# lucabaldesi/srsRAN

Measured on AMD Instinct MI355X. Metric: PDSCH decoded Mbps + code-blocks/sec, 20 MHz TM4 QAM256, 1/2/4/8 GPU, higher is better.
Workload: dtype fp32+int16; 1 GPU; srslte_ue_dl chain from time-domain I/Q: 2048 subframes/GPU/batch, 20 MHz (100 PRB), TM4 2x2 spatial multiplexing, 2 codewords QAM256 TBS 97896 (C=16, K=6144), MMSE+CSI, max 10 half-its with CRC early stop, 40 dB crossed 2x2 channel, every subframe distinct (GPU eNodeB generator, keyed by global subframe index); 3 PHY worker threads (own ue_dl / stream / softbuffers each) decode alternate batches,; subframes_per_gpu_batch=2048, code_blocks_per_gpu_batch=65536, workers_per_gpu=3, parallelism=dp1

## Files before the change

srsran_amd/csrc/tdec_internal.h:

```cpp
#pragma once
#include <hip/hip_runtime.h>
#include <stdint.h>

#include "dlsch_internal.h"

#define TDEC_INF 10000
#define TDEC_WARMUP 40
#define TDEC_SEG 8

namespace mi355 {

struct TdecWinArgs {
  const int16_t*  in;
  size_t          in_stride;
  const uint32_t* in_idx;
  const uint8_t*  done;
  const uint32_t* remaining;
  uint32_t*       A1;
  uint32_t*       E;
  uint32_t*       D;
  uint32_t*       ckpt;
  const uint32_t* dstE;
  const uint32_t* dstA;
  int             ncb, L, Lp, nseg, n, write_d;
  uint8_t*        dec;
  size_t          dec_stride;
  const uint32_t* gS;
  const uint32_t* gP;
  DlschCheckArgs  chk;
  int             chk_on;
  int             spec;
  int             rowmask;
};

struct TdecDecideArgs {
  const uint32_t* D;
  uint8_t*        out;
  size_t          out_stride;
  int             ncb, L, Lp;
  const uint8_t*  done;
  const uint32_t* remaining;
};

struct TdecGenArgs {
  const uint32_t* S;
  const uint32_t* P0;
  const uint32_t* P1;
  uint32_t*       A1;
  uint32_t*       E;
  uint32_t*       D;
  uint32_t*       ckpt;
  const uint16_t* pi;
  int             npair, K, Kp, nseg, n, write_d;
};

struct TdecGenPrepArgs {
  const int16_t*  in;
  size_t          stride;
  const uint32_t* in_idx;
  uint32_t *     S, *P0, *P1, *E;
  int            ncb, npair, K, Kp;
};

struct TdecGenDecideArgs {
  const uint32_t* D;
  uint8_t*        out;
  size_t          out_stride;
  int             ncb, K, Kp;
};

#define TDEC_GEN_CB_L 12
#define TDEC_GEN_CB_KP(K) (((K) + 3 + 7) / 8 * 8)
struct TdecGenCbArgs {
  const int16_t*  in;
  size_t          in_stride;
  const uint32_t* in_idx;
  uint16_t*       ws;
  const uint16_t* pi;
  uint8_t*        out;
  size_t          out_stride;
  uint32_t*       reruns;
  int             ncb, K, Kp, h0, h1, warm, persist;
};
int        tdec_gen_cb_threads(int K);
size_t     tdec_gen_cb_lds(int K, int threads);
hipError_t tdec_gen_cb_launch(const TdecGenCbArgs& a, hipStream_t s);

struct TdecLatArgs {
  const int16_t*  in;
  size_t          in_stride;
  const uint32_t* in_idx;
  const uint32_t* dstE;
  const uint32_t* dstA;
  uint8_t*        done;
  DlschCheckArgs  chk;
  uint64_t*       prof;
  int             ncb, K, rowmask;
  int             bwave;
  int             owaves;
};
size_t     tdec_lat_lds(int K, int nsb);
hipError_t tdec_lat_launch(int nsb, const TdecLatArgs& a, hipStream_t s);

struct TdecRun {
  const int16_t*  in;
  size_t          in_stride;
  const uint32_t* in_idx;
  const uint8_t*  done;
  const uint32_t* remaining;
  uint32_t        n, K, h0, h1;
  uint8_t*        out;
  size_t          out_stride;
  hipStream_t     stream;
  const DlschCheckArgs* chk = nullptr;
  bool*                 chk_fused = nullptr;
  bool  spec       = false;
  bool* spec_taken = nullptr;
  bool  redo       = false;
  bool  rowmask    = false;
};

hipError_t tdec_win_launch_halfit(int nsb, const TdecWinArgs& a, hipStream_t s);
bool       tdec_win_spec_ok(int nsb, int L);
int        tdec_set_diag(int mode);
hipError_t tdec_win_launch_decide(int nsb, const TdecDecideArgs& a, hipStream_t s);
hipError_t tdec_gen_launch_prep(const TdecGenPrepArgs& a, hipStream_t s);
hipError_t tdec_gen_launch_halfit(const TdecGenArgs& a, hipStream_t s);
hipError_t tdec_gen_launch_decide(const TdecGenDecideArgs& a, hipStream_t s);

}

struct mi355_tdec_batch;
int mi355_tdec_run_internal(mi355_tdec_batch* q, const mi355::TdecRun& r);
int mi355_tdec_win_tables(mi355_tdec_batch* q, uint32_t K, const uint32_t** dstE, const uint32_t** dstA);
```

srsran_amd/csrc/tdec_kernels.hip:

```cpp
#include <hip/hip_runtime.h>

#include <atomic>
#include <stdint.h>
#include <stdlib.h>

#include "crc_device.h"
#include "tdec_internal.h"
#include "tdec_trellis.h"

namespace mi355 {

__device__ __forceinline__ uint32_t hi_lo(uint32_t a, uint32_t b) { return __builtin_amdgcn_alignbit(b, a, 16); }
__device__ __forceinline__ uint32_t from_prev(uint32_t v)
{
  return (uint32_t)__builtin_amdgcn_update_dpp(0, (int)v, 0x111, 0xf, 0xf, true);
}
__device__ __forceinline__ uint32_t from_next(uint32_t v)
{
  return (uint32_t)__builtin_amdgcn_update_dpp(0, (int)v, 0x101, 0xf, 0xf, true);
}

__device__ __forceinline__ void bm_set(uint32_t* bm, uint32_t m, bool v)
{
  const uint32_t by = m >> 3;
  if (v) atomicOr(&bm[by >> 2], 1u << (((by & 3) << 3) + 7 - (m & 7)));
}

template <int NL>
__device__ __forceinline__ void tdec_fused_check(const TdecWinArgs& a, int cb, int l, int K, const uint32_t* bm,
                                                 const uint32_t (*t4)[4][256])
{
  const DlschCheckArgs& c      = a.chk;
  const CbDesc&         d      = c.desc[cb];
  const uint32_t        nbytes = (uint32_t)K / 8, chunk = nbytes / NL;
  const int             pi     = d.C > 1 ? 1 : 0;
  const uint8_t*        bytes  = (const uint8_t*)bm;
  uint32_t              crc    = crc24_words(bytes + l * chunk, chunk, t4[pi]);
  crc = gf2_mulmod24(crc, c.scale[128 + 8 * pi + l], pi ? c.crc24b->poly : c.crc24a->poly);
#pragma unroll
  for (int o = NL / 2; o >= 1; o >>= 1) crc ^= (uint32_t)__shfl_xor((int)crc, o, 64);
  const bool ok  = crc == 0;
  const bool fin = ok || c.h + 1 == c.max_its;
  if (fin) {
    uint8_t*       dst  = c.data + d.data_off + (size_t)d.cb * d.rlen / 8;
    const uint32_t nb   = d.nb;
    const uint32_t head = min(nb, (4u - (uint32_t)((uintptr_t)dst & 3u)) & 3u);
    const uint32_t nw   = (nb - head) / 4, tail0 = head + 4 * nw;
    for (uint32_t i = l; i < head; i += NL) dst[i] = bytes[i];
    for (uint32_t i = tail0 + l; i < nb; i += NL) dst[i] = bytes[i];
    uint32_t* dw = (uint32_t*)(dst + head);
    const uint32_t sh = head;
    for (uint32_t w = l; w < nw; w += NL) {
      const uint32_t lo = bm[w + sh / 4], hi = bm[w + sh / 4 + 1];
      dw[w]             = sh ? __builtin_amdgcn_alignbyte(hi, lo, sh) : lo;
    }
    if (l == 0) {
      c.its[cb] = c.h + 1;
      if (ok) {
        c.done[cb]       = 1;
        c.sb_crc[d.slot] = 1;
      } else {
        c.done[cb] = 2;
      }
    }
  }
  const uint64_t un = __builtin_amdgcn_ballot_w64(l == 0 && !fin);
  if (un && (threadIdx.x & 63) == (uint32_t)__builtin_ctzll(un)) flag_set(c.next);
}


#define WG_AT(arr, j) (arr)[((size_t)grp * Lp + (j)) * 64 + q]

#define TDEC_BM_WORDS (8 * 193)
__shared__ uint32_t tdec_tx_lds[4][2][TDEC_SEG * 64];
__shared__ uint32_t tdec_ym_lds[4][8 * SB_ROWMASK_WORDS];
__shared__ uint32_t tdec_bm_lds[4 * TDEC_BM_WORDS];
__shared__ int16_t  tdec_stg_lds[4][TDEC_SEG * 128];
__shared__ uint32_t tdec_stg_row[4][TDEC_SEG];

#ifndef TDEC_WAVES_PER_EU
#define TDEC_WAVES_PER_EU 2
#endif
template <int NSB, int SEG, int MODE, int DIAG, bool FULL, int OUTK, bool GI = false, bool TX = false>
__device__ __forceinline__ void tdec_win_body(const TdecWinArgs& a, const int gl,
                                              const uint32_t (*crc_t4)[4][256] = nullptr)
{
  constexpr int NL = NSB / 2;
  constexpr int G  = 64 / NL;
  static_assert(!TX || (NSB == 16 && FULL && SEG == 8), "TX loads need 8-lane rows and whole 8-step segments");
  static_assert((DIAG >= 0 && DIAG <= 4) || DIAG == 20, "DIAG values the body knows");
  const int     grp = __builtin_amdgcn_readfirstlane(gl >> 6), q = gl & 63;
  const int     cbg = q / NL, l = q % NL;
  if constexpr (!TX) {
    if (grp * G + cbg >= a.ncb) return;
    if (a.done && a.done[grp * G + cbg]) return;
  }
  if (a.remaining && *a.remaining == 0) return;

  const int  L = a.L, Lp = a.Lp, nseg = a.nseg;
  constexpr bool CL     = DIAG == 20;
  constexpr bool dec2   = MODE == 2;
  constexpr bool has_ap = MODE == 1;

  const int       cb   = grp * G + cbg;
  const int       K    = L * NSB;
  const size_t    bidx = a.in_idx ? a.in_idx[cb] : (size_t)cb;
  const uint32_t* in32 = (const uint32_t*)(a.in + bidx * a.in_stride);
  const size_t    wg0  = (size_t)grp * Lp * 64 + q;
  const uint32_t* X    = dec2 ? a.E + wg0 : (GI ? a.gS + wg0 : in32 + l);
  const int       xs   = (dec2 || GI) ? 64 : NL;
  const uint32_t* Y    = GI ? a.gP + wg0 : in32 + (dec2 ? (K + 32) : (K + 32) / 2) + l;
  const int       ys   = GI ? 64 : NL;
  const uint32_t* AP   = a.A1 + wg0;
  uint32_t*       ck   = a.ckpt + (size_t)grp * nseg * 8 * 64 + q;

  const uint4*    txin  = nullptr;
  if constexpr (TX) {
    const int txc = grp * G + ((q >> 1) & 7);
    txin = (const uint4*)(a.in + (a.in_idx ? (size_t)a.in_idx[txc] : (size_t)txc) * a.in_stride) + (2 * (q >> 4) + (q & 1));
  }
  const int       txoX  = 0;
  const int       txoY  = (dec2 ? (L * NSB + 32) : (L * NSB + 32) / 2) / 4;
  uint32_t*       txb   = nullptr;
  if constexpr (TX) {
    txb = &tdec_tx_lds[threadIdx.x >> 6][0][0];
  }
  constexpr bool RMK = NSB == 16 && !GI;
  uint32_t*      ymask = nullptr;
  if constexpr (RMK) {
    ymask = tdec_ym_lds[threadIdx.x >> 6];
#pragma unroll
    for (int w = l; w < SB_ROWMASK_WORDS; w += NL) {
      uint32_t v = 0xffffffffu;
      if (a.rowmask) v = ((const uint32_t*)(a.in + bidx * a.in_stride + SB_ROWMASK))[(dec2 ? SB_ROWMASK_WORDS : 0) + w];
      ymask[cbg * SB_ROWMASK_WORDS + w] = v;
    }
    __builtin_amdgcn_fence(__ATOMIC_RELEASE, "wavefront");
    __builtin_amdgcn_wave_barrier();
    __builtin_amdgcn_fence(__ATOMIC_ACQUIRE, "wavefront");
  }
  auto yrow = [&](int c, int j) -> bool {
    if constexpr (RMK) {
      return (ymask[c * SB_ROWMASK_WORDS + (j >> 5)] >> (j & 31)) & 1u;
    } else {
      return true;
    }
  };
  auto tx_load = [&](int so, int j0, uint32_t* r, bool par = false) {
    uint4 v0 = make_uint4(0u, 0u, 0u, 0u), v1 = v0;
    const int tc = (q >> 1) & 7, jr = j0 + (q >> 4);
    if (!par || yrow(tc, jr)) v0 = txin[so + j0 * 2];
    if (!par || yrow(tc, jr + 4)) v1 = txin[so + (j0 + 4) * 2];
    r[0] = v0.x; r[1] = v0.y; r[2] = v0.z; r[3] = v0.w;
    r[4] = v1.x; r[5] = v1.y; r[6] = v1.z; r[7] = v1.w;
  };
  auto tx_unpack = [&](int b, const uint32_t* r, uint32_t* o) {
    uint32_t* w = txb + b * SEG * 64;
    ((uint4*)w)[q]      = make_uint4(r[0], r[1], r[2], r[3]);
    ((uint4*)w)[64 + q] = make_uint4(r[4], r[5], r[6], r[7]);
    __builtin_amdgcn_fence(__ATOMIC_RELEASE, "wavefront");
    __builtin_amdgcn_wave_barrier();
    __builtin_amdgcn_fence(__ATOMIC_ACQUIRE, "wavefront");
#pragma unroll
    for (int i = 0; i < SEG; i++) o[i] = w[64 * i + q];
  };

  v2s st[8], nw[8], aw[8];

  set_minf(aw);
#pragma unroll 1
  for (int b = 0; b < TDEC_WARMUP / 8; b++) {
    uint32_t xo[8], yo[8], ao[8] = {};
#pragma unroll
    for (int i = 0; i < 8; i++) {
      const int j = (L - TDEC_WARMUP) + 8 * b + i;
      xo[i]       = X[j * xs];
      yo[i]       = yrow(cbg, j) ? Y[j * ys] : 0u;
      if constexpr (has_ap) ao[i] = AP[j * 64];
    }
#pragma unroll
    for (int i = 0; i < 8; i++) {
      const int k = 8 * b + i;
      v2s       x = U(hi_lo(from_prev(xo[i]), xo[i]));
      if constexpr (has_ap) x = sadd(x, U(hi_lo(from_prev(ao[i]), ao[i])));
      if constexpr (CL) {
        aw[k & 7] = aw[k & 7] ^ x ^ U(yo[i]);
        continue;
      }
      v2s c0[8], c1[8];
      alpha_cands<true>(aw, x, U(hi_lo(from_prev(yo[i]), yo[i])), c0, c1);
#pragma unroll
      for (int s = 0; s < 8; s++) aw[s] = vmax(c0[s], c1[s]);
      if ((k & 1) == 0 && k != 0) normalize<true>(aw);
    }
  }

  if constexpr (DIAG != 2) {
  set_minf(st);
#pragma unroll 1
  for (int b = TDEC_WARMUP / 8 - 1; b >= 0; b--) {
    uint32_t xo[8], yo[8], ao[8] = {};
#pragma unroll
    for (int i = 0; i < 8; i++) {
      const int j = 8 * b + i;
      xo[i]       = X[j * xs];
      yo[i]       = yrow(cbg, j) ? Y[j * ys] : 0u;
      if constexpr (has_ap) ao[i] = AP[j * 64];
    }
#pragma unroll
    for (int i = 7; i >= 0; i--) {
      const int k = 8 * b + i;
      v2s       x = U(hi_lo(xo[i], from_next(xo[i])));
      if constexpr (has_ap) x = sadd(x, U(hi_lo(ao[i], from_next(ao[i]))));
      if constexpr (CL) {
        st[k & 7] = st[k & 7] ^ x ^ U(yo[i]);
        continue;
      }
      beta_step<true>(st, x, U(hi_lo(yo[i], from_next(yo[i]))), nw);
#pragma unroll
      for (int s = 0; s < 8; s++) st[s] = nw[s];
      if ((k & 1) == 0 && k != 0) normalize<true>(st);
    }
  }
  if (l == NL - 1) {
    const int16_t* T = a.in + bidx * a.in_stride + 3 * (K + 32) + (dec2 ? 6 : 0);
    v2s            tr[8], tn[8];
    tr[0] = splat(0);
#pragma unroll
    for (int i = 1; i < 8; i++) tr[i] = splat(-TDEC_INF);
#pragma unroll
    for (int t = 2; t >= 0; t--) {
      beta_step<false>(tr, splat(T[2 * t]), splat(T[2 * t + 1]), tn);
#pragma unroll
      for (int i = 0; i < 8; i++) tr[i] = tn[i];
    }
#pragma unroll
    for (int i = 0; i < 8; i++) st[i] = (v2s){st[i].x, tr[i].y};
  }
#pragma unroll
  for (int s = 0; s < 8; s++) ck[((size_t)(nseg - 1) * 8 + s) * 64] = W(st[s]);

  {
    uint32_t cx[SEG], cy[SEG], ca[SEG] = {};
    auto     load = [&](int t, uint32_t* x, uint32_t* y, uint32_t* ap) {
      if constexpr (TX) {
        if constexpr (!dec2) tx_load(txoX, t * SEG, x);
        tx_load(txoY, t * SEG, y, true);
      }
#pragma unroll
      for (int i = 0; i < SEG; i++) {
        const int j = FULL ? t * SEG + i : min(t * SEG + i, L - 1);
        if constexpr (!TX || dec2) x[i] = X[j * xs];
        if constexpr (!TX) y[i] = yrow(cbg, j) ? Y[j * ys] : 0u;
        if constexpr (has_ap) ap[i] = AP[j * 64];
      }
    };
    uint32_t bx[SEG], by[SEG], ba[SEG] = {}, dx[SEG], dy[SEG], da[SEG] = {};
    load(nseg - 1, cx, cy, ca);
    if (nseg > 1) load(nseg - 2, bx, by, ba);
    auto seg = [&](int t, const uint32_t* rx, const uint32_t* ry, const uint32_t* sa, uint32_t* lx, uint32_t* ly,
                   uint32_t* la) {
      uint32_t sx[SEG], sy[SEG];
      if constexpr (TX) {
        if constexpr (!dec2) tx_unpack(0, rx, sx);
        tx_unpack(1, ry, sy);
      }
#pragma unroll
      for (int i = 0; i < SEG; i++) {
        if constexpr (!TX || dec2) sx[i] = rx[i];
        if constexpr (!TX) sy[i] = ry[i];
      }
      if (t > 1) load(t - 2, lx, ly, la);
#pragma unroll
      for (int i = SEG - 1; i >= 0; i--) {
        const int k = t * SEG + i;
        if (FULL || k < L) {
          v2s x = U(sx[i]);
          if constexpr (has_ap) x = sadd(x, U(sa[i]));
          if constexpr (DIAG == 4) {
            st[0] = st[0] ^ x ^ U(sy[i]);
            continue;
          }
          if constexpr (CL) {
            st[i] = st[i] ^ x ^ U(sy[i]);
          } else {
            beta_step<true>(st, x, U(sy[i]), nw);
#pragma unroll
            for (int s = 0; s < 8; s++) st[s] = nw[s];
          }
          if (i == 0 && t > 0 && DIAG != 3) {
#pragma unroll
            for (int s = 0; s < 8; s++) ck[((size_t)(t - 1) * 8 + s) * 64] = W(st[s]);
          }
          if (!CL && (i & 1) == 0 && k != 0) normalize<true>(st);
        }
      }
    };
#pragma unroll 1
    for (int t = nseg - 1; t >= 0; t -= 3) {
      seg(t, cx, cy, ca, dx, dy, da);
      if (t >= 1) seg(t - 1, bx, by, ba, cx, cy, ca);
      if (t >= 2) seg(t - 2, dx, dy, da, bx, by, ba);
    }
  }
  }
  if constexpr (DIAG == 1 || DIAG == 3 || DIAG == 4) {
    if (st[0].x == 12345 && st[1].y == 777) a.D[q] = W(st[0]);
    return;
  }
#pragma unroll
  for (int s = 0; s < 8; s++) st[s] = aw[s];
  if (l == 0) {
    st[0].x = 0;
#pragma unroll
    for (int i = 1; i < 8; i++) st[i].x = -TDEC_INF;
  }

  int16_t*        E16  = (int16_t*)a.E + (size_t)grp * Lp * 128;
  int16_t*        A16  = (int16_t*)a.A1 + (size_t)grp * Lp * 128;
  int16_t*        D16  = (int16_t*)a.D + (size_t)grp * Lp * 128;
  const uint32_t* tab  = (dec2 ? a.dstA : a.dstE) + l;
  const int       lane0 = cbg * NL;
  constexpr bool  dec_o   = OUTK == 1 || OUTK == 3;
  constexpr bool  wr_bits = !dec2 && dec_o && FULL;
  constexpr bool  wr_bm   = dec_o && (dec2 || !FULL);
  constexpr bool  wr_d    = OUTK == 2;
  constexpr bool  wr_a1   = !(dec2 && OUTK == 3);
  constexpr bool  wr_e    = !(!dec2 && OUTK == 3);
  constexpr int BMW = NSB == 16 ? 193 : 25;
  uint32_t*     bm  = nullptr;
  if constexpr (dec2 || wr_bits || wr_bm) {
    static_assert(G * BMW <= TDEC_BM_WORDS, "decision bitmaps of a wave");
    bm = tdec_bm_lds + (threadIdx.x >> 6) * TDEC_BM_WORDS + cbg * BMW;
    if constexpr (wr_bm) {
      for (int w = l; w < K / 32; w += NL) bm[w] = 0;
      __builtin_amdgcn_fence(__ATOMIC_RELEASE, "wavefront");
      __builtin_amdgcn_wave_barrier();
    }
  }

  constexpr bool STG = FULL && !GI && (dec2 ? wr_a1 : wr_e);
  int16_t*       O16 = dec2 ? A16 : E16;
  int16_t*       stg = nullptr;
  uint32_t*      stg_row = nullptr;
  if constexpr (STG) {
    stg     = tdec_stg_lds[threadIdx.x >> 6];
    stg_row = tdec_stg_row[threadIdx.x >> 6];
  }
  auto put = [&](int i, uint32_t tb, v2s v) {
    if constexpr (STG) {
      stg[i * 128 + (tb & 127u) + 2 * lane0]         = v.x;
      stg[i * 128 + ((tb >> 16) & 127u) + 2 * lane0] = v.y;
      stg_row[i]                                     = (tb & 0xffffu) >> 7;
    } else {
      O16[(tb & 0xffffu) + lane0 * 2] = v.x;
      O16[(tb >> 16) + lane0 * 2]     = v.y;
    }
  };
  auto flush = [&]() {
    if constexpr (STG) {
      static_assert(SEG == 8 && NL % 4 == 0, "rows of 8 steps, whole 16-byte pieces per code block");
      constexpr int PPR = NL / 4;
      __builtin_amdgcn_fence(__ATOMIC_RELEASE, "wavefront");
      __builtin_amdgcn_wave_barrier();
      __builtin_amdgcn_fence(__ATOMIC_ACQUIRE, "wavefront");
#pragma unroll
      for (int k = 0; k < 2; k++) {
        const int      idx = k * NL + l, r = idx / PPR, pc = idx % PPR;
        const uint32_t jr  = stg_row[r];
        const uint4    v   = *(const uint4*)(stg + r * 128 + 2 * lane0 + pc * 8);
        *(uint4*)(O16 + (size_t)jr * 128 + 2 * lane0 + pc * 8) = v;
      }
      __builtin_amdgcn_fence(__ATOMIC_RELEASE, "wavefront");
      __builtin_amdgcn_wave_barrier();
    }
  };
  uint32_t cx[SEG], cy[SEG], ca[SEG] = {}, cd[SEG], cc[8];
  auto     load = [&](int t, uint32_t* x, uint32_t* y, uint32_t* ap, uint32_t* d, uint32_t* c) {
    if constexpr (TX) {
      if constexpr (!dec2) tx_load(txoX, t * SEG, x);
      tx_load(txoY, t * SEG, y, true);
    }
#pragma unroll
    for (int i = 0; i < SEG; i++) {
      const int j = FULL ? t * SEG + i : min(t * SEG + i, L - 1);
      if constexpr (!TX || dec2) x[i] = X[j * xs];
      if constexpr (!TX) y[i] = yrow(cbg, j) ? Y[j * ys] : 0u;
      if constexpr (has_ap) ap[i] = AP[j * 64];
      d[i] = tab[(size_t)j * NL];
    }
#pragma unroll
    for (int s = 0; s < 8; s++) c[s] = ck[((size_t)t * 8 + s) * 64];
  };
  load(0, cx, cy, ca, cd, cc);

  uint32_t nx[SEG], ny[SEG], na[SEG] = {}, nd[SEG], nc[8];
  auto fseg = [&](int t, const uint32_t* rx, const uint32_t* ry, const uint32_t* ca, const uint32_t* cd,
                  const uint32_t* cc, uint32_t* nx, uint32_t* ny, uint32_t* na, uint32_t* nd, uint32_t* nc) {
    uint32_t cx[SEG], cy[SEG];
    if constexpr (TX) {
      if constexpr (!dec2) tx_unpack(0, rx, cx);
      tx_unpack(1, ry, cy);
    }
#pragma unroll
    for (int i = 0; i < SEG; i++) {
      if constexpr (!TX || dec2) cx[i] = rx[i];
      if constexpr (!TX) cy[i] = ry[i];
    }
    const int s0 = t * SEG;
    const int e  = FULL ? s0 + SEG : ((s0 + SEG < L) ? s0 + SEG : L);
    uint32_t  bits = 0;
    if (t + 1 < nseg) load(t + 1, nx, ny, na, nd, nc);

    v2s xin[SEG];
#pragma unroll
    for (int i = 0; i < SEG; i++) {
      if constexpr (has_ap) {
        xin[i] = sadd(U(cx[i]), U(ca[i]));
      } else {
        xin[i] = U(cx[i]);
      }
    }

    static_assert(SEG == 8, "the rebuild keeps the 8 rows of a segment in registers");
    v2s ck8[8];
#pragma unroll
    for (int s = 0; s < 8; s++) ck8[s] = U(cc[s]);
    if constexpr (CL) {
#pragma unroll
      for (int i = 0; i < SEG; i++) {
        const int j = s0 + i;
        if (FULL ? i < SEG : j < e) {
          const v2s      out = xin[i] ^ U(cy[i]) ^ ck8[i] ^ st[i];
          const uint32_t tb  = cd[i];
          if constexpr (!dec2) {
            if constexpr (wr_e) put(i, tb, out);
            bits |= ((uint32_t)(out.x > 0) << (15 - i)) | ((uint32_t)(out.y > 0) << (7 - i));
            if constexpr (wr_bm) {
              bm_set(bm, 2 * l * L + j, out.x > 0);
              bm_set(bm, (2 * l + 1) * L + j, out.y > 0);
            }
          } else {
            if constexpr (wr_a1) put(i, tb, out);
            if constexpr (wr_bm) {
              const uint32_t jd = (tb & 0xffffu) >> 7, wlo = tb & 15u, whi = (tb >> 16) & 15u;
              bm_set(bm, wlo * L + jd, out.x > 0);
              bm_set(bm, whi * L + jd, out.y > 0);
            }
          }
        }
      }
    } else {
      v2s        cur[8], R[8][8];
      const bool ck_norm = (e & 1) == 0 && e != L;
#pragma unroll
      for (int s = 0; s < 8; s++) cur[s] = ck8[s];
      if (ck_norm) normalize<true>(cur);
#pragma unroll
      for (int i = SEG; i >= 1; i--) {
        const int j = s0 + i;
        if (FULL ? i == SEG : j == e) {
#pragma unroll
          for (int s = 0; s < 8; s++) R[i - 1][s] = ck8[s];
        } else if (FULL ? i < SEG : j < e) {
          v2s row[8];
          beta_step<true>(cur, xin[i], U(cy[i]), row);
#pragma unroll
          for (int s = 0; s < 8; s++) cur[s] = row[s];
#pragma unroll
          for (int s = 0; s < 8; s++) R[i - 1][s] = row[s];
          if ((j & 1) == 0) normalize<true>(cur);
        }
      }
#pragma unroll
      for (int i = 0; i < SEG; i++) {
        const int j = s0 + i;
        if (FULL ? i < SEG : j < e) {
          v2s c0[8], c1[8];
          alpha_cands<true>(st, xin[i], U(cy[i]), c0, c1);
          v2s t0[8], t1[8];
#pragma unroll
          for (int s = 0; s < 8; s++) {
            t0[s] = sadd(R[i][s], c0[s]);
            t1[s] = sadd(R[i][s], c1[s]);
          }
          const v2s m0 = vmax(vmax(vmax(t0[0], t0[1]), vmax(t0[2], t0[3])), vmax(vmax(t0[4], t0[5]), vmax(t0[6], t0[7])));
          const v2s m1 = vmax(vmax(vmax(t1[0], t1[1]), vmax(t1[2], t1[3])), vmax(vmax(t1[4], t1[5]), vmax(t1[6], t1[7])));
          const v2s out = ssub(m1, m0);
#pragma unroll
          for (int s = 0; s < 8; s++) st[s] = vmax(c0[s], c1[s]);
          if ((i & 1) == 0 && j != 0) normalize<true>(st);

          const uint32_t tb  = cd[i];
          const uint32_t olo = (tb & 0xffffu) + lane0 * 2, ohi = (tb >> 16) + lane0 * 2;
          if constexpr (!dec2) {
            if constexpr (wr_e) put(i, tb, has_ap ? out - U(ca[i]) : out);
            if constexpr (wr_d) WG_AT(a.D, j) = W(out);
            bits |= ((uint32_t)(out.x > 0) << (15 - i)) | ((uint32_t)(out.y > 0) << (7 - i));
            if constexpr (wr_bm) {
              bm_set(bm, 2 * l * L + j, out.x > 0);
              bm_set(bm, (2 * l + 1) * L + j, out.y > 0);
            }
          } else {
            if constexpr (wr_a1) put(i, tb, out - xin[i]);
            if constexpr (wr_bm) {
              const uint32_t jd = (tb & 0xffffu) >> 7, wlo = tb & 15u, whi = (tb >> 16) & 15u;
              bm_set(bm, wlo * L + jd, out.x > 0);
              bm_set(bm, whi * L + jd, out.y > 0);
            }
            if constexpr (wr_d) {
              D16[olo] = out.x;
              D16[ohi] = out.y;
            }
          }
        }
      }
    }
    flush();
    if constexpr (wr_bits) {
      uint8_t* bb = (uint8_t*)bm + (size_t)(2 * l) * (L / 8) + t;
      bb[0]       = (uint8_t)(bits >> 8);
      bb[L / 8]   = (uint8_t)bits;
    }
  };
#pragma unroll 1
  for (int t = 0; t < nseg; t += 2) {
    fseg(t, cx, cy, ca, cd, cc, nx, ny, na, nd, nc);
    if (t + 1 < nseg) fseg(t + 1, nx, ny, na, nd, nc, cx, cy, ca, cd, cc);
  }
  if constexpr (wr_bm || wr_bits) {
    __builtin_amdgcn_fence(__ATOMIC_RELEASE, "wavefront");
    __builtin_amdgcn_wave_barrier();
    __builtin_amdgcn_fence(__ATOMIC_ACQUIRE, "wavefront");
    if (crc_t4) {
      tdec_fused_check<NL>(a, cb, l, K, bm, crc_t4);
    } else {
      uint2* o = (uint2*)(a.dec + (size_t)cb * a.dec_stride);
      for (int w = l; w < K / 64; w += NL) o[w] = make_uint2(bm[2 * w], bm[2 * w + 1]);
    }
  }
}

template <int NSB, int SEG, int MODE, int DIAG = 0, bool FULL = false, int OUTK = 0, bool TX = false>
__global__ __launch_bounds__(256) __attribute__((amdgpu_waves_per_eu(TDEC_WAVES_PER_EU))) void tdec_win_halfit(TdecWinArgs a)
{
  const int gl = blockIdx.x * blockDim.x + threadIdx.x;
  const uint32_t (*t4)[4][256] = nullptr;
  if constexpr (OUTK == 1 || OUTK == 3) {
    __shared__ uint32_t crc_t4[2][4][256];
    if (a.chk_on) {
      if (a.remaining && *a.remaining == 0) return;
      const uint32_t ti = threadIdx.x;
      crc_t4[0][0][ti] = a.chk.crc24a->t[ti];
      crc_t4[1][0][ti] = a.chk.crc24b->t[ti];
      __syncthreads();
#pragma unroll
      for (int k = 1; k < 4; k++) {
        crc_t4[0][k][ti] = crc24_step_table(crc_t4[0][k - 1][ti], crc_t4[0][0]);
        crc_t4[1][k][ti] = crc24_step_table(crc_t4[1][k - 1][ti], crc_t4[1][0]);
        __syncthreads();
      }
      t4 = crc_t4;
    }
  }
  if constexpr (TX) {
    const int  cb  = (gl >> 6) * (128 / NSB) + (gl & 63) / (NSB / 2);
    const bool act = cb < a.ncb && !(a.done && a.done[cb]);
    if (__builtin_amdgcn_ballot_w64(act) == ~0ull) {
      tdec_win_body<NSB, SEG, MODE, DIAG, FULL, OUTK, false, true>(a, gl, t4);
      return;
    }
  }
  tdec_win_body<NSB, SEG, MODE, DIAG, FULL, OUTK>(a, gl, t4);
}


template <int NSB>
__global__ __launch_bounds__(256) void tdec_win_decide_rows(TdecDecideArgs a)
{
  constexpr int NL = NSB / 2;
  constexpr int G  = 64 / NL;
  const size_t  g  = (size_t)blockIdx.x * blockDim.x + threadIdx.x;
  const int     q  = (int)(g & 63);
  const size_t  r  = g >> 6;
  const int     nb = a.L / 8;
  const int     grp = (int)(r / nb), jb = (int)(r % nb);
  const int     cbg = q / NL, l = q % NL;
  const size_t  cb  = (size_t)grp * G + cbg;
  if (cb >= (size_t)a.ncb || (a.remaining && *a.remaining == 0) || (a.done && a.done[cb])) return;
  const uint32_t* D  = a.D + ((size_t)grp * a.Lp + 8 * jb) * 64 + q;
  uint32_t        lo = 0, hi = 0;
#pragma unroll
  for (int i = 0; i < 8; i++) {
    const v2s v = U(D[(size_t)i * 64]);
    lo |= (uint32_t)(v.x > 0) << (7 - i);
    hi |= (uint32_t)(v.y > 0) << (7 - i);
  }
  uint8_t* o = a.out + cb * a.out_stride;
  o[(2 * l) * nb + jb]     = (uint8_t)lo;
  o[(2 * l + 1) * nb + jb] = (uint8_t)hi;
}

template <int NSB>
__global__ __launch_bounds__(256) void tdec_win_decide(TdecDecideArgs a)
{
  constexpr int NL   = NSB / 2;
  constexpr int G    = 64 / NL;
  const size_t  g    = (size_t)blockIdx.x * blockDim.x + threadIdx.x;
  const int     K    = a.L * NSB;
  const int     nbyt = K / 8;
  const size_t  cb   = g / nbyt;
  if (cb >= (size_t)a.ncb || (a.remaining && *a.remaining == 0) || (a.done && a.done[cb])) return;
  const int      b   = (int)(g % nbyt);
  const int      grp = (int)(cb / G), cbg = (int)(cb % G);
  const int16_t* D16 = (const int16_t*)a.D + (size_t)grp * a.Lp * 128 + cbg * NL * 2;
  uint32_t       out = 0;
#pragma unroll
  for (int i = 0; i < 8; i++) {
    const int nat = 8 * b + i, w = nat / a.L, j = nat % a.L;
    out |= (uint32_t)(D16[(size_t)j * 128 + w] > 0) << (7 - i);
  }
  a.out[cb * a.out_stride + b] = (uint8_t)out;
}


static std::atomic<int> g_diag{-1};

static int diag_mode()
{
  int v = g_diag.load(std::memory_order_relaxed);
  if (v < 0) {
    const char* e = getenv("MI355_TDEC_DIAG");
    v             = e ? atoi(e) : 0;
    g_diag.store(v, std::memory_order_relaxed);
  }
  return v;
}

int tdec_set_diag(int mode)
{
  const int old = diag_mode();
  g_diag.store(mode < 0 ? 0 : mode, std::memory_order_relaxed);
  return old;
}

static size_t diag_lds()
{
  static const long m = getenv("MI355_TDEC_LDS") ? atol(getenv("MI355_TDEC_LDS")) : 0;
  return (size_t)m;
}

template <int NSB, int DIAG, bool FULL, int OUTK, bool TX = false>
static void launch_mode_t(int mode, int blocks, const TdecWinArgs& a, hipStream_t s)
{
  const size_t lds = diag_lds();
  if (mode == 0) {
    hipLaunchKernelGGL((tdec_win_halfit<NSB, TDEC_SEG, 0, DIAG, FULL, OUTK, TX>), dim3(blocks), dim3(256), lds, s, a);
  } else if (mode == 1) {
    hipLaunchKernelGGL((tdec_win_halfit<NSB, TDEC_SEG, 1, DIAG, FULL, OUTK, TX>), dim3(blocks), dim3(256), lds, s, a);
  } else {
    hipLaunchKernelGGL((tdec_win_halfit<NSB, TDEC_SEG, 2, DIAG, FULL, OUTK, TX>), dim3(blocks), dim3(256), lds, s, a);
  }
}

static bool tx_enabled()
{
  static const bool on = !getenv("MI355_TDEC_TX") || atoi(getenv("MI355_TDEC_TX")) != 0;
  return on;
}

template <int NSB, int DIAG, bool FULL, int OUTK>
static void launch_mode_o(int mode, int blocks, const TdecWinArgs& a, hipStream_t s)
{
  if constexpr (NSB == 16 && FULL && (DIAG == 0 || DIAG == 20)) {
    if (tx_enabled() && (uintptr_t)a.in % 16 == 0 && (a.in_stride * sizeof(int16_t)) % 16 == 0 && (a.L * 16 + 32) % 16 == 0) {
      launch_mode_t<NSB, DIAG, FULL, OUTK, true>(mode, blocks, a, s);
      return;
    }
  }
  launch_mode_t<NSB, DIAG, FULL, OUTK>(mode, blocks, a, s);
}

template <int NSB, int DIAG, bool FULL = false>
static void launch_mode(int mode, int blocks, const TdecWinArgs& a, hipStream_t s)
{
  if constexpr (NSB == 16 && FULL && DIAG == 0) {
    if (a.dec && a.spec) {
      launch_mode_o<NSB, DIAG, FULL, 3>(mode, blocks, a, s);
      return;
    }
  }
  if (a.dec) {
    launch_mode_o<NSB, DIAG, FULL, 1>(mode, blocks, a, s);
  } else if (a.write_d) {
    launch_mode_o<NSB, DIAG, FULL, 2>(mode, blocks, a, s);
  } else {
    launch_mode_o<NSB, DIAG, FULL, 0>(mode, blocks, a, s);
  }
}

bool tdec_win_spec_ok(int nsb, int L) { return nsb == 16 && L % TDEC_SEG == 0 && diag_mode() == 0; }

hipError_t tdec_win_launch_halfit(int nsb, const TdecWinArgs& a, hipStream_t s)
{
  const int ngrp   = (a.ncb + (128 / nsb) - 1) / (128 / nsb);
  const int blocks = (ngrp * 64 + 255) / 256;
  const int mode   = (a.n & 1) ? 2 : (a.n > 0 ? 1 : 0);
  const int dm     = diag_mode();
  if (nsb == 16) {
    if (dm == 1) {
      launch_mode<16, 1>(mode, blocks, a, s);
    } else if (dm == 3) {
      launch_mode<16, 3>(mode, blocks, a, s);
    } else if (dm == 4) {
      launch_mode<16, 4>(mode, blocks, a, s);
    } else if (dm == 2) {
      launch_mode<16, 2>(mode, blocks, a, s);
    } else if (dm == 20 && a.L % TDEC_SEG == 0) {
      launch_mode<16, 20, true>(mode, blocks, a, s);
    } else if (a.L % TDEC_SEG == 0) {
      launch_mode<16, 0, true>(mode, blocks, a, s);
    } else {
      launch_mode<16, 0>(mode, blocks, a, s);
    }
  } else if (a.L % TDEC_SEG == 0) {
    launch_mode<8, 0, true>(mode, blocks, a, s);
  } else {
    launch_mode<8, 0>(mode, blocks, a, s);
  }
  return hipGetLastError();
}

hipError_t tdec_win_launch_decide(int nsb, const TdecDecideArgs& a, hipStream_t s)
{
  if (a.L % 8 == 0) {
    const int    G      = 128 / nsb;
    const size_t ngrp   = (a.ncb + G - 1) / G;
    const size_t total  = ngrp * (a.L / 8) * 64;
    const int    blocks = (int)((total + 255) / 256);
    if (nsb == 16) {
      hipLaunchKernelGGL(tdec_win_decide_rows<16>, dim3(blocks), dim3(256), 0, s, a);
    } else {
      hipLaunchKernelGGL(tdec_win_decide_rows<8>, dim3(blocks), dim3(256), 0, s, a);
    }
    return hipGetLastError();
  }
  const size_t total  = (size_t)a.ncb * (a.L * nsb / 8);
  const int    blocks = (int)((total + 255) / 256);
  if (nsb == 16) {
    hipLaunchKernelGGL(tdec_win_decide<16>, dim3(blocks), dim3(256), 0, s, a);
  } else {
    hipLaunchKernelGGL(tdec_win_decide<8>, dim3(blocks), dim3(256), 0, s, a);
  }
  return hipGetLastError();
}

}
```

srsran_amd/csrc/tdec_runtime.cpp:

```cpp
#include <hip/hip_runtime.h>

#include <map>
#include <mutex>
#include <stdio.h>
#include <string.h>
#include <vector>

#include "../../include/srsran_amd/tdec.h"
#include "device_mem.h"
#include "lte_qpp_table.h"
#include "tdec_internal.h"

using namespace mi355;

namespace {

int cb_index(uint32_t K)
{
  for (int i = 0; i < LTE_NOF_CB_SIZES; i++) {
    if (lte_qpp_table[i][0] == K) return i;
    if (lte_qpp_table[i][0] > K) break;
  }
  return -1;
}

uint32_t round_up(uint32_t v, uint32_t m) { return (v + m - 1) / m * m; }

struct KTables {
  DevMem dstE, dstA;
  DevMem pi;
};

struct Geometry {
  uint32_t K, nsb, L, Lp, nl, nseg, ngrp;
  uint32_t npair, Kp;
};

Geometry geometry(uint32_t K, uint32_t ncb, int impl)
{
  Geometry g{};
  g.K   = K;
  g.nsb = impl == MI355_TDEC_GENERIC ? 0 : mi355_tdec_autoimp_get_subblocks(K);
  if (g.nsb) {
    g.L    = K / g.nsb;
    g.Lp   = round_up(g.L, TDEC_SEG);
    g.nl   = g.nsb / 2;
    g.nseg = (g.L + TDEC_SEG - 1) / TDEC_SEG;
    g.ngrp = (ncb + (64 / g.nl) - 1) / (64 / g.nl);
  } else {
    g.npair = (ncb + 1) / 2;
    g.Kp    = round_up(K + 3, TDEC_SEG);
    g.nseg  = (K + TDEC_SEG - 1) / TDEC_SEG;
  }
  return g;
}

}

struct mi355_tdec_batch {
  int                          device = 0;
  hipStream_t                  own    = nullptr;
  DevScratch                   ws;
  DevCache<uint32_t, KTables>  tables;
  DevCache<uint32_t, KTables>  gtables;
  int                          impl = MI355_TDEC_AUTO;
  int                          gen_cb   = -1;
  int                          gen_warm = 32;
  DevMem                       reruns;
  bool                         prof = false;
  std::vector<hipEvent_t>      ev;
  size_t                       ev_used = 0;
  std::mutex                   mu;
};

static int get_tables(mi355_tdec_batch_t* q, const Geometry& g, KTables** out)
{
  return (g.nsb ? q->tables : q->gtables).get(g.K, out, [&](KTables& t) -> int {
    const uint32_t K   = g.K;
    const int      idx = cb_index(K);
    if (idx < 0) return MI355_ERROR_INVALID_INPUTS;
    const uint64_t        f1 = lte_qpp_table[idx][1], f2 = lte_qpp_table[idx][2];
    std::vector<uint16_t> pi(K), inv(K);
    for (uint64_t m = 0; m < K; m++) {
      pi[m]       = (uint16_t)((f1 * m + f2 * m * m) % K);
      inv[pi[m]]  = (uint16_t)m;
    }
    if (g.nsb) {
      std::vector<uint32_t> dE((size_t)g.L * g.nl, 0), dA((size_t)g.L * g.nl, 0);
      for (uint32_t j = 0; j < g.L; j++) {
        for (uint32_t l = 0; l < g.nl; l++) {
          uint32_t n0 = (2 * l) * g.L + j, n1 = (2 * l + 1) * g.L + j;
          uint32_t e0 = inv[n0], e1 = inv[n1], a0 = pi[n0], a1 = pi[n1];
          if (e0 % g.L != e1 % g.L || a0 % g.L != a1 % g.L) return MI355_ERROR;
          dE[(size_t)j * g.nl + l] = ((e0 % g.L) * 128 + e0 / g.L) | (((e1 % g.L) * 128 + e1 / g.L) << 16);
          dA[(size_t)j * g.nl + l] = ((a0 % g.L) * 128 + a0 / g.L) | (((a1 % g.L) * 128 + a1 / g.L) << 16);
        }
      }
      CHECK_HIP(t.dstE.upload(dE));
      CHECK_HIP(t.dstA.upload(dA));
    } else {
      std::vector<uint16_t> both(pi);
      both.insert(both.end(), inv.begin(), inv.end());
      CHECK_HIP(t.pi.upload(both));
    }
    return MI355_SUCCESS;
  });
}

static size_t ws_bytes(const Geometry& g, uint32_t n, bool cbk = false)
{
  if (cbk) return (size_t)n * 5 * TDEC_GEN_CB_KP(g.K) * 2 + 256;
  if (g.nsb) {
    const size_t arr = (size_t)g.ngrp * g.Lp * 64 * 4;
    static const size_t pad = getenv("MI355_TDEC_WS_PAD") ? (size_t)atoll(getenv("MI355_TDEC_WS_PAD")) : 0;
    return 3 * (arr + pad) + (size_t)g.ngrp * g.nseg * 8 * 64 * 4 + 8 * 256 + 3 * 256;
  }
  const size_t arr = (size_t)g.npair * g.Kp * 4;
  return 6 * arr + (size_t)g.npair * 16 + (size_t)g.npair * g.nseg * 32 + 8 * 256;
}

static int ensure_ws(mi355_tdec_batch_t* q, size_t bytes)
{
  CHECK_HIP(q->ws.reserve(bytes, bytes + bytes / 8, DevScratch::SyncFree));
  return MI355_SUCCESS;
}

static hipEvent_t next_event(mi355_tdec_batch_t* q)
{
  if (q->ev_used == q->ev.size()) {
    hipEvent_t e;
    if (hipEventCreate(&e) != hipSuccess) return nullptr;
    q->ev.push_back(e);
  }
  return q->ev[q->ev_used++];
}

extern "C" {

uint32_t mi355_tdec_autoimp_get_subblocks(uint32_t long_cb)
{
  if (!(long_cb % 16) && long_cb > 800) return 16;
  if (!(long_cb % 8) && long_cb > 400) return 8;
  return 0;
}

int mi355_tdec_batch_create(mi355_tdec_batch_t** q, int device)
{
  if (!q) return MI355_ERROR_INVALID_INPUTS;
  int ndev = 0;
  CHECK_HIP(hipGetDeviceCount(&ndev));
  if (device < 0 || device >= ndev) return MI355_ERROR_INVALID_INPUTS;
  CHECK_HIP(hipSetDevice(device));
  auto* b   = new mi355_tdec_batch;
  b->device = device;
  if (hipStreamCreateWithFlags(&b->own, hipStreamNonBlocking) != hipSuccess) {
    delete b;
    return MI355_ERROR;
  }
  *q = b;
  return MI355_SUCCESS;
}

void mi355_tdec_batch_destroy(mi355_tdec_batch_t* q)
{
  if (!q) return;
  (void)hipSetDevice(q->device);
  (void)hipDeviceSynchronize();
  for (auto e : q->ev) (void)hipEventDestroy(e);
  if (q->own) (void)hipStreamDestroy(q->own);
  delete q;
}

int mi355_tdec_set_diag(int mode) { return mi355::tdec_set_diag(mode); }

void mi355_tdec_batch_set_profiling(mi355_tdec_batch_t* q, int enable)
{
  if (q) q->prof = enable != 0;
}

int mi355_tdec_batch_kernel_stats(mi355_tdec_batch_t* q, double* ms, uint32_t* launches)
{
  if (!q) return MI355_ERROR_INVALID_INPUTS;
  double total = 0;
  for (size_t i = 0; i + 1 < q->ev_used; i += 2) {
    CHECK_HIP(hipEventSynchronize(q->ev[i + 1]));
    float t = 0;
    CHECK_HIP(hipEventElapsedTime(&t, q->ev[i], q->ev[i + 1]));
    total += t;
  }
  if (ms) *ms = total;
  if (launches) *launches = (uint32_t)(q->ev_used / 2);
  q->ev_used = 0;
  return MI355_SUCCESS;
}

}

int mi355_tdec_win_tables(mi355_tdec_batch_t* q, uint32_t K, const uint32_t** dstE, const uint32_t** dstA)
{
  if (!q || cb_index(K) < 0 || mi355_tdec_autoimp_get_subblocks(K) == 0) return MI355_ERROR_INVALID_INPUTS;
  std::lock_guard<std::mutex> lock(q->mu);
  const Geometry g = geometry(K, 1, MI355_TDEC_AUTO);
  KTables*       t = nullptr;
  const int      r = get_tables(q, g, &t);
  if (r) return r;
  *dstE = t->dstE.as<uint32_t>();
  *dstA = t->dstA.as<uint32_t>();
  return MI355_SUCCESS;
}

int mi355_tdec_run_internal(mi355_tdec_batch_t* q, const TdecRun& rq)
{
  const int16_t* d_in = rq.in;
  size_t in_stride = rq.in_stride;
  uint32_t n = rq.n, K = rq.K, h0 = rq.h0, h1 = rq.h1;
  uint8_t* d_out = rq.out;
  size_t out_stride = rq.out_stride;
  if (!q || !d_in || !d_out || h1 <= h0 || cb_index(K) < 0) return MI355_ERROR_INVALID_INPUTS;
  const bool generic = q->impl == MI355_TDEC_GENERIC || mi355_tdec_autoimp_get_subblocks(K) == 0;
  const size_t need  = generic ? 3 * (size_t)K + 12 : 3 * (size_t)(K + 32) + 12;
  if (in_stride < need || (in_stride & 1) || out_stride < K / 8) {
    return MI355_ERROR_INVALID_INPUTS;
  }
  if (n == 0) return MI355_SUCCESS;
  std::lock_guard<std::mutex> lock(q->mu);
  CHECK_HIP(hipSetDevice(q->device));
  hipStream_t s = rq.stream ? rq.stream : q->own;

  const Geometry g = geometry(K, n, q->impl);
  if (rq.redo && !g.nsb) return MI355_SUCCESS;
  KTables*       t = nullptr;
  int            r = get_tables(q, g, &t);
  if (r) return r;
  const bool cbk = !g.nsb && !rq.done && !rq.remaining && !rq.chk &&
                   (q->gen_cb == 1 || (q->gen_cb < 0 && (K > 400 || n <= 4096)));
  if (h0 == 0) {
    if ((r = ensure_ws(q, ws_bytes(g, n, cbk)))) return r;
  } else if (ws_bytes(g, n, cbk) > q->ws.cap()) {
    return MI355_ERROR;
  }

  char* p     = q->ws.base();
  auto  carve = [&](size_t bytes) {
    char* c = p;
    p += ((bytes + 255) / 256) * 256;
    return c;
  };

  if (g.nsb) {
    const size_t arr = (size_t)g.ngrp * g.Lp * 64 * 4;
    static const size_t pad = getenv("MI355_TDEC_WS_PAD") ? (size_t)atoll(getenv("MI355_TDEC_WS_PAD")) : 0;
    auto*        A1  = (uint32_t*)carve(arr + pad);
    auto*        E   = (uint32_t*)carve(arr + pad);
    auto*        D   = (uint32_t*)carve(arr + pad);
    auto*        CK  = (uint32_t*)carve((size_t)g.ngrp * g.nseg * 8 * 64 * 4);

    const bool fuse = (g.L % 8 == 0 || (K % 64 == 0 && (K / 8) % (g.nsb / 2) == 0)) && out_stride % 8 == 0 &&
                      (uintptr_t)d_out % 8 == 0;
    const uint32_t *dstE = t->dstE.as<uint32_t>(), *dstA = t->dstA.as<uint32_t>();
    for (uint32_t h = h0; h < h1; h++) {
      if (rq.redo) {
        TdecWinArgs wa{d_in, in_stride, rq.in_idx, rq.done, rq.remaining, A1, E, D, CK, dstE, dstA,
                       (int)n, (int)g.L, (int)g.Lp, (int)g.nseg, (int)h, 0, nullptr, out_stride};
        wa.rowmask = rq.rowmask && g.nsb == 16 && in_stride == SB_STRIDE;
        CHECK_HIP(tdec_win_launch_halfit(g.nsb, wa, s));
        continue;
      }
      TdecWinArgs wa{d_in, in_stride, rq.in_idx, rq.done, rq.remaining, A1, E, D, CK, dstE, dstA,
                     (int)n, (int)g.L, (int)g.Lp, (int)g.nseg, (int)h, h + 1 == h1,
                     (fuse && h + 1 == h1) ? d_out : nullptr, out_stride};
      wa.rowmask = rq.rowmask && g.nsb == 16 && in_stride == SB_STRIDE;
      if (rq.spec && fuse && h + 1 == h1 && tdec_win_spec_ok(g.nsb, g.L)) {
        wa.spec = 1;
        if (rq.spec_taken) *rq.spec_taken = true;
      }
      if (rq.chk && fuse && h + 1 == h1) {
        wa.chk    = *rq.chk;
        wa.chk.h  = h;
        wa.chk_on = 1;
        if (rq.chk_fused) *rq.chk_fused = true;
      }
      hipEvent_t e0 = nullptr, e1 = nullptr;
      if (q->prof) {
        e0 = next_event(q);
        e1 = next_event(q);
        if (e0) (void)hipEventRecord(e0, s);
      }
      CHECK_HIP(tdec_win_launch_halfit(g.nsb, wa, s));
      if (q->prof && e1) (void)hipEventRecord(e1, s);
    }
    if (!fuse && !rq.redo) {
      TdecDecideArgs da{D, d_out, out_stride, (int)n, (int)g.L, (int)g.Lp, rq.done, rq.remaining};
      CHECK_HIP(tdec_win_launch_decide(g.nsb, da, s));
    }
  } else if (cbk) {
    TdecGenCbArgs ca{};
    ca.in         = d_in;
    ca.in_stride  = in_stride;
    ca.in_idx     = rq.in_idx;
    ca.ws         = (uint16_t*)q->ws.base();
    ca.pi         = t->pi.as<uint16_t>();
    ca.out        = d_out;
    ca.out_stride = out_stride;
    ca.reruns     = q->reruns.as<uint32_t>();
    ca.ncb        = (int)n;
    ca.K          = (int)K;
    ca.Kp         = TDEC_GEN_CB_KP((int)K);
    ca.h0         = (int)h0;
    ca.h1         = (int)h1;
    ca.warm       = q->gen_warm;
    ca.persist    = 1;
    hipEvent_t e0 = nullptr, e1 = nullptr;
    if (q->prof) {
      e0 = next_event(q);
      e1 = next_event(q);
      if (e0) (void)hipEventRecord(e0, s);
    }
    CHECK_HIP(tdec_gen_cb_launch(ca, s));
    if (q->prof && e1) (void)hipEventRecord(e1, s);
  } else {
    const size_t arr = (size_t)g.npair * g.Kp * 4;
    auto*        S   = (uint32_t*)carve(arr);
    auto*        P0  = (uint32_t*)carve(arr);
    auto*        P1  = (uint32_t*)carve(arr);
    auto*        A1  = (uint32_t*)carve(arr);
    auto*        E   = (uint32_t*)carve(arr);
    auto*        D   = (uint32_t*)carve(arr);
    auto*        CK  = (uint32_t*)carve((size_t)g.npair * g.nseg * 32);

    if (h0 == 0) {
      TdecGenPrepArgs pa{d_in, in_stride, rq.in_idx, S, P0, P1, E, (int)n, (int)g.npair, (int)K, (int)g.Kp};
      CHECK_HIP(tdec_gen_launch_prep(pa, s));
    }
    for (uint32_t h = h0; h < h1; h++) {
      TdecGenArgs ga{S, P0, P1, A1, E, D, CK, t->pi.as<uint16_t>(),
                     (int)g.npair, (int)K, (int)g.Kp, (int)g.nseg, (int)h, h + 1 == h1};
      hipEvent_t e0 = nullptr, e1 = nullptr;
      if (q->prof) {
        e0 = next_event(q);
        e1 = next_event(q);
        if (e0) (void)hipEventRecord(e0, s);
      }
      CHECK_HIP(tdec_gen_launch_halfit(ga, s));
      if (q->prof && e1) (void)hipEventRecord(e1, s);
    }
    TdecGenDecideArgs da{D, d_out, out_stride, (int)n, (int)K, (int)g.Kp};
    CHECK_HIP(tdec_gen_launch_decide(da, s));
  }
  return MI355_SUCCESS;
}

extern "C" {

int mi355_tdec_batch_run_dev(mi355_tdec_batch_t* q,
                             const int16_t*      d_in,
                             size_t              in_stride,
                             uint32_t            n,
                             uint32_t            K,
                             uint32_t            nhalf,
                             uint8_t*            d_out,
                             size_t              out_stride,
                             void*               stream)
{
  if (nhalf == 0) return MI355_ERROR_INVALID_INPUTS;
  return mi355_tdec_run_internal(
      q, TdecRun{d_in, in_stride, nullptr, nullptr, nullptr, n, K, 0, nhalf, d_out, out_stride, (hipStream_t)stream});
}

int mi355_tdec_batch_halfit_dev(mi355_tdec_batch_t* q,
                                const int16_t*      d_in,
                                size_t              in_stride,
                                uint32_t            n,
                                uint32_t            K,
                                uint32_t            half_idx,
                                uint8_t*            d_out,
                                size_t              out_stride,
                                void*               stream)
{
  return mi355_tdec_run_internal(q, TdecRun{d_in, in_stride, nullptr, nullptr, nullptr, n, K, half_idx, half_idx + 1, d_out,
                                            out_stride, (hipStream_t)stream});
}

int mi355_tdec_batch_set_generic(mi355_tdec_batch_t* q, int per_cb, int warmup)
{
  if (!q || per_cb < -1 || per_cb > 1 || warmup < 0) return MI355_ERROR_INVALID_INPUTS;
  std::lock_guard<std::mutex> lock(q->mu);
  q->gen_cb   = per_cb;
  q->gen_warm = warmup;
  return MI355_SUCCESS;
}

int mi355_tdec_batch_generic_reruns(mi355_tdec_batch_t* q, uint32_t* reruns)
{
  if (!q || !reruns) return MI355_ERROR_INVALID_INPUTS;
  std::lock_guard<std::mutex> lock(q->mu);
  CHECK_HIP(hipSetDevice(q->device));
  if (!q->reruns.p) {
    CHECK_HIP(q->reruns.alloc(4));
    CHECK_HIP(hipMemset(q->reruns.p, 0, 4));
    *reruns = 0;
    return MI355_SUCCESS;
  }
  CHECK_HIP(hipDeviceSynchronize());
  CHECK_HIP(hipMemcpy(reruns, q->reruns.p, 4, hipMemcpyDeviceToHost));
  CHECK_HIP(hipMemset(q->reruns.p, 0, 4));
  return MI355_SUCCESS;
}

int mi355_tdec_batch_set_impl(mi355_tdec_batch_t* q, int impl)
{
  if (!q || (impl != MI355_TDEC_AUTO && impl != MI355_TDEC_GENERIC)) return MI355_ERROR_INVALID_INPUTS;
  q->impl = impl;
  return MI355_SUCCESS;
}

int mi355_tdec_batch_run(mi355_tdec_batch_t* q,
                         const int16_t*      in,
                         size_t              in_stride,
                         uint32_t            n,
                         uint32_t            K,
                         uint32_t            nhalf,
                         uint8_t*            out,
                         size_t              out_stride)
{
  if (!q || !in || !out) return MI355_ERROR_INVALID_INPUTS;
  if (n == 0) return MI355_SUCCESS;
  CHECK_HIP(hipSetDevice(q->device));
  DevMem din, dout;
  CHECK_HIP(din.alloc((size_t)n * in_stride * 2));
  CHECK_HIP(dout.alloc((size_t)n * out_stride));
  CHECK_HIP(hipMemcpyAsync(din.p, in, (size_t)n * in_stride * 2, hipMemcpyHostToDevice, q->own));
  int r = mi355_tdec_batch_run_dev(q, din.as<int16_t>(), in_stride, n, K, nhalf, dout.as<uint8_t>(), out_stride,
                                   q->own);
  if (r == MI355_SUCCESS) {
    CHECK_HIP(hipMemcpyAsync(out, dout.p, (size_t)n * out_stride, hipMemcpyDeviceToHost, q->own));
    CHECK_HIP(hipStreamSynchronize(q->own));
  }
  return r;
}

void* mi355_dev_alloc(size_t bytes, int device)
{
  void* p = nullptr;
  if (hipSetDevice(device) != hipSuccess) return nullptr;
  if (hipMalloc(&p, bytes) != hipSuccess) return nullptr;
  return p;
}

void mi355_dev_free(void* p)
{
  if (p) (void)hipFree(p);
}

}

static int device_of(const void* p, int* dev)
{
  hipPointerAttribute_t a{};
  if (hipPointerGetAttributes(&a, p) != hipSuccess) {
    (void)hipGetLastError();
    return -1;
  }
  if (a.type != hipMemoryTypeDevice && a.type != hipMemoryTypeManaged) return -1;
  *dev = a.device;
  return 0;
}

static int sync_device_of(const void* p)
{
  int cur = 0, dev = 0;
  CHECK_HIP(hipGetDevice(&cur));
  if (device_of(p, &dev)) dev = cur;
  if (dev != cur) CHECK_HIP(hipSetDevice(dev));
  const hipError_t e = hipDeviceSynchronize();
  if (dev != cur) (void)hipSetDevice(cur);
  return e == hipSuccess ? MI355_SUCCESS : MI355_ERROR;
}

extern "C" {

int mi355_memcpy_h2d(void* dst, const void* src, size_t bytes)
{
  if (!bytes) return MI355_SUCCESS;
  if (sync_device_of(dst)) return MI355_ERROR;
  CHECK_HIP(hipMemcpy(dst, src, bytes, hipMemcpyHostToDevice));
  return sync_device_of(dst);
}

int mi355_memcpy_d2h(void* dst, const void* src, size_t bytes)
{
  if (!bytes) return MI355_SUCCESS;
  if (sync_device_of(src)) return MI355_ERROR;
  CHECK_HIP(hipMemcpy(dst, src, bytes, hipMemcpyDeviceToHost));
  return MI355_SUCCESS;
}

int mi355_memset_dev(void* dst, int value, size_t bytes)
{
  if (!bytes) return MI355_SUCCESS;
  if (sync_device_of(dst)) return MI355_ERROR;
  CHECK_HIP(hipMemset(dst, value, bytes));
  return sync_device_of(dst);
}

int mi355_device_sync(void)
{
  CHECK_HIP(hipDeviceSynchronize());
  return MI355_SUCCESS;
}

int mi355_device_count(void)
{
  int n = 0;
  if (hipGetDeviceCount(&n) != hipSuccess) return 0;
  return n;
}

}
```

Measured before the change: 126,700 Mbps.

## Hoist turbo-decoder segment prefetch above warmup and make loads branch-free

The backward-recursion segment loads now start before the beta warmup loop, so their memory latency overlaps the warmup computation. Row-masked parity loads become unconditional reads from a device-resident zero buffer selected by pointer, which removes divergent branches around the vector loads. The segment loop gets a steady-state body with unconditional prefetch plus a tail, and sched_barrier and waitcnt hints are added. In exchange it uses more registers (more live prefetch buffers), does redundant clamped loads at the tail, and requires allocating a zero buffer per batch object.

```diff
diff --git a/srsran_amd/csrc/tdec_internal.h b/srsran_amd/csrc/tdec_internal.h
--- a/srsran_amd/csrc/tdec_internal.h
+++ b/srsran_amd/csrc/tdec_internal.h
@@ -31,6 +31,7 @@
   int             chk_on;
   int             spec;
   int             rowmask;
+  const uint4*    zero16;
 };
 
 struct TdecDecideArgs {
diff --git a/srsran_amd/csrc/tdec_kernels.hip b/srsran_amd/csrc/tdec_kernels.hip
--- a/srsran_amd/csrc/tdec_kernels.hip
+++ b/srsran_amd/csrc/tdec_kernels.hip
@@ -147,10 +147,16 @@
     }
   };
   auto tx_load = [&](int so, int j0, uint32_t* r, bool par = false) {
-    uint4 v0 = make_uint4(0u, 0u, 0u, 0u), v1 = v0;
-    const int tc = (q >> 1) & 7, jr = j0 + (q >> 4);
-    if (!par || yrow(tc, jr)) v0 = txin[so + j0 * 2];
-    if (!par || yrow(tc, jr + 4)) v1 = txin[so + (j0 + 4) * 2];
+    const int    tc = (q >> 1) & 7, jr = j0 + (q >> 4);
+    const uint4* p0 = txin + so + j0 * 2;
+    const uint4* p1 = txin + so + (j0 + 4) * 2;
+    if constexpr (RMK) {
+      if (par) {
+        p0 = yrow(tc, jr) ? p0 : a.zero16;
+        p1 = yrow(tc, jr + 4) ? p1 : a.zero16;
+      }
+    }
+    const uint4 v0 = *p0, v1 = *p1;
     r[0] = v0.x; r[1] = v0.y; r[2] = v0.z; r[3] = v0.w;
     r[4] = v1.x; r[5] = v1.y; r[6] = v1.z; r[7] = v1.w;
   };
@@ -196,6 +202,23 @@
   }
 
   if constexpr (DIAG != 2) {
+  uint32_t cx[SEG], cy[SEG], ca[SEG] = {};
+  auto     load = [&](int t, uint32_t* x, uint32_t* y, uint32_t* ap) {
+    if constexpr (TX) {
+      if constexpr (!dec2) tx_load(txoX, t * SEG, x);
+      tx_load(txoY, t * SEG, y, true);
+    }
+#pragma unroll
+    for (int i = 0; i < SEG; i++) {
+      const int j = FULL ? t * SEG + i : min(t * SEG + i, L - 1);
+      if constexpr (!TX || dec2) x[i] = X[j * xs];
+      if constexpr (!TX) y[i] = yrow(cbg, j) ? Y[j * ys] : 0u;
+      if constexpr (has_ap) ap[i] = AP[j * 64];
+    }
+  };
+  uint32_t bx[SEG], by[SEG], ba[SEG] = {}, dx[SEG], dy[SEG], da[SEG] = {};
+  load(nseg - 1, cx, cy, ca);
+  load(max(nseg - 2, 0), bx, by, ba);
   set_minf(st);
 #pragma unroll 1
   for (int b = TDEC_WARMUP / 8 - 1; b >= 0; b--) {
@@ -241,26 +264,10 @@
   for (int s = 0; s < 8; s++) ck[((size_t)(nseg - 1) * 8 + s) * 64] = W(st[s]);
 
   {
-    uint32_t cx[SEG], cy[SEG], ca[SEG] = {};
-    auto     load = [&](int t, uint32_t* x, uint32_t* y, uint32_t* ap) {
-      if constexpr (TX) {
-        if constexpr (!dec2) tx_load(txoX, t * SEG, x);
-        tx_load(txoY, t * SEG, y, true);
-      }
-#pragma unroll
-      for (int i = 0; i < SEG; i++) {
-        const int j = FULL ? t * SEG + i : min(t * SEG + i, L - 1);
-        if constexpr (!TX || dec2) x[i] = X[j * xs];
-        if constexpr (!TX) y[i] = yrow(cbg, j) ? Y[j * ys] : 0u;
-        if constexpr (has_ap) ap[i] = AP[j * 64];
-      }
-    };
-    uint32_t bx[SEG], by[SEG], ba[SEG] = {}, dx[SEG], dy[SEG], da[SEG] = {};
-    load(nseg - 1, cx, cy, ca);
-    if (nseg > 1) load(nseg - 2, bx, by, ba);
-    auto seg = [&](int t, const uint32_t* rx, const uint32_t* ry, const uint32_t* sa, uint32_t* lx, uint32_t* ly,
-                   uint32_t* la) {
+    auto seg = [&](int t, bool pf, const uint32_t* rx, const uint32_t* ry, const uint32_t* sa, uint32_t* lx,
+                   uint32_t* ly, uint32_t* la) {
       uint32_t sx[SEG], sy[SEG];
+      __builtin_amdgcn_sched_barrier(0);
       if constexpr (TX) {
         if constexpr (!dec2) tx_unpack(0, rx, sx);
         tx_unpack(1, ry, sy);
@@ -270,7 +277,7 @@
         if constexpr (!TX || dec2) sx[i] = rx[i];
         if constexpr (!TX) sy[i] = ry[i];
       }
-      if (t > 1) load(t - 2, lx, ly, la);
+      if (pf) load(max(t - 2, 0), lx, ly, la);
 #pragma unroll
       for (int i = SEG - 1; i >= 0; i--) {
         const int k = t * SEG + i;
@@ -296,12 +303,15 @@
         }
       }
     };
+    int t = nseg - 1;
 #pragma unroll 1
-    for (int t = nseg - 1; t >= 0; t -= 3) {
-      seg(t, cx, cy, ca, dx, dy, da);
-      if (t >= 1) seg(t - 1, bx, by, ba, cx, cy, ca);
-      if (t >= 2) seg(t - 2, dx, dy, da, bx, by, ba);
-    }
+    for (; t >= 2; t -= 3) {
+      seg(t, true, cx, cy, ca, dx, dy, da);
+      seg(t - 1, true, bx, by, ba, cx, cy, ca);
+      seg(t - 2, true, dx, dy, da, bx, by, ba);
+    }
+    if (t >= 0) seg(t, false, cx, cy, ca, dx, dy, da);
+    if (t >= 1) seg(t - 1, false, bx, by, ba, cx, cy, ca);
   }
   }
   if constexpr (DIAG == 1 || DIAG == 3 || DIAG == 4) {
@@ -398,6 +408,7 @@
   auto fseg = [&](int t, const uint32_t* rx, const uint32_t* ry, const uint32_t* ca, const uint32_t* cd,
                   const uint32_t* cc, uint32_t* nx, uint32_t* ny, uint32_t* na, uint32_t* nd, uint32_t* nc) {
     uint32_t cx[SEG], cy[SEG];
+    __builtin_amdgcn_sched_barrier(0);
     if constexpr (TX) {
       if constexpr (!dec2) tx_unpack(0, rx, cx);
       tx_unpack(1, ry, cy);
@@ -410,7 +421,7 @@
     const int s0 = t * SEG;
     const int e  = FULL ? s0 + SEG : ((s0 + SEG < L) ? s0 + SEG : L);
     uint32_t  bits = 0;
-    if (t + 1 < nseg) load(t + 1, nx, ny, na, nd, nc);
+    load(min(t + 1, nseg - 1), nx, ny, na, nd, nc);
 
     v2s xin[SEG];
 #pragma unroll
@@ -523,6 +534,7 @@
       bb[L / 8]   = (uint8_t)bits;
     }
   };
+  __builtin_amdgcn_s_waitcnt(0x0f70);
 #pragma unroll 1
   for (int t = 0; t < nseg; t += 2) {
     fseg(t, cx, cy, ca, cd, cc, nx, ny, na, nd, nc);
@@ -673,7 +685,7 @@
 static void launch_mode_o(int mode, int blocks, const TdecWinArgs& a, hipStream_t s)
 {
   if constexpr (NSB == 16 && FULL && (DIAG == 0 || DIAG == 20)) {
-    if (tx_enabled() && (uintptr_t)a.in % 16 == 0 && (a.in_stride * sizeof(int16_t)) % 16 == 0 && (a.L * 16 + 32) % 16 == 0) {
+    if (tx_enabled() && a.zero16 && (uintptr_t)a.in % 16 == 0 && (a.in_stride * sizeof(int16_t)) % 16 == 0 && (a.L * 16 + 32) % 16 == 0) {
       launch_mode_t<NSB, DIAG, FULL, OUTK, true>(mode, blocks, a, s);
       return;
     }
diff --git a/srsran_amd/csrc/tdec_runtime.cpp b/srsran_amd/csrc/tdec_runtime.cpp
--- a/srsran_amd/csrc/tdec_runtime.cpp
+++ b/srsran_amd/csrc/tdec_runtime.cpp
@@ -67,6 +67,7 @@
   int                          gen_cb   = -1;
   int                          gen_warm = 32;
   DevMem                       reruns;
+  DevMem                       zero16;
   bool                         prof = false;
   std::vector<hipEvent_t>      ev;
   size_t                       ev_used = 0;
@@ -153,7 +154,9 @@
   CHECK_HIP(hipSetDevice(device));
   auto* b   = new mi355_tdec_batch;
   b->device = device;
-  if (hipStreamCreateWithFlags(&b->own, hipStreamNonBlocking) != hipSuccess) {
+  const std::vector<uint32_t> zero(64, 0u);
+  if (hipStreamCreateWithFlags(&b->own, hipStreamNonBlocking) != hipSuccess || b->zero16.upload(zero) != hipSuccess) {
+    if (b->own) (void)hipStreamDestroy(b->own);
     delete b;
     return MI355_ERROR;
   }
@@ -263,6 +266,7 @@
         TdecWinArgs wa{d_in, in_stride, rq.in_idx, rq.done, rq.remaining, A1, E, D, CK, dstE, dstA,
                        (int)n, (int)g.L, (int)g.Lp, (int)g.nseg, (int)h, 0, nullptr, out_stride};
         wa.rowmask = rq.rowmask && g.nsb == 16 && in_stride == SB_STRIDE;
+        wa.zero16  = q->zero16.as<uint4>();
         CHECK_HIP(tdec_win_launch_halfit(g.nsb, wa, s));
         continue;
       }
@@ -270,6 +274,7 @@
                      (int)n, (int)g.L, (int)g.Lp, (int)g.nseg, (int)h, h + 1 == h1,
                      (fuse && h + 1 == h1) ? d_out : nullptr, out_stride};
       wa.rowmask = rq.rowmask && g.nsb == 16 && in_stride == SB_STRIDE;
+      wa.zero16  = q->zero16.as<uint4>();
       if (rq.spec && fuse && h + 1 == h1 && tdec_win_spec_ok(g.nsb, g.L)) {
         wa.spec = 1;
         if (rq.spec_taken) *rq.spec_taken = true;
```

New measurement: 130,200 Mbps, median of 6. 1.03x the previous value.
